# madeleineudell/LowRankModels.jl

Measured on AMD Instinct MI355X. Metric: observed-entry updates/sec, higher is better.
Workload: dtype f64

## Files before the change

### lowrankmodels.jl_amd/csrc/glrm_cached.hip

```cpp
#include <hip/hip_runtime.h>

#include <algorithm>
#include <atomic>
#include <vector>

#include "glrm_device.hpp"
#include "glrm_engine.hpp"
#include "glrm_launch.hpp"

using namespace glrm;

namespace {

struct CachedArgs {
  int64_t nseg;
  const int64_t* ptr;
  const int32_t* idx;
  const double* vals;
  double* own;
  int64_t own_offset;
  const double* other;
  double* alpha;
  const glrm_loss* losses;
  const glrm_reg* regs;
  int reg_single;
  int k;
  double fixed_alpha;
  double min_stepsize;
  int32_t* trials;
  int32_t* accepts;
  int cap;
  const int32_t* seglist;
  int64_t seg_lo, seg_hi;
  int vecreg;
};

__device__ __forceinline__ int64_t cached_segment(const CachedArgs& a, int64_t slot) {
  if (slot >= a.nseg) return -1;
  if (!a.seglist) return slot;
  const int64_t seg = a.seglist[slot];
  return (seg < a.seg_lo || seg >= a.seg_hi) ? -1 : seg;
}

template <int G, int R, int LOSS, bool GRAD>
__device__ __forceinline__ double cached_pass(const CachedArgs& a, const char* __restrict__ ybuf, const double* __restrict__ lval,
                                              const int32_t* __restrict__ lidx, const Vec<G, R>& xv, Vec<G, R>& g, int len, int gi, int j,
                                              const LossDesc& segloss) {
  constexpr int KPB = G * R * 8, NG = 64 / G, LM = loss_mode(LOSS), U = 4;
  constexpr bool TRIG = loss_trig(LOSS);
  double J = 0.0;
  if (GRAD) {
#pragma unroll
    for (int i = 0; i < R / 2; ++i) g.v[i] = make_double2(0.0, 0.0);
  }
  for (int t0 = 0; t0 < len; t0 += NG * U) {
    double2 y[U][R / 2];
    double av[U];
    int cc[U];
    bool valid[U];
#pragma unroll
    for (int u = 0; u < U; ++u) {
      const int t = t0 + u * NG + gi;
      valid[u] = t < len;
      const int tt = valid[u] ? t : len - 1;
      const char* yp = ybuf + tt * KPB + j * 16;
#pragma unroll
      for (int i = 0; i < R / 2; ++i) y[u][i] = *reinterpret_cast<const double2*>(yp + i * (G * 16));
      av[u] = lval[tt];
      cc[u] = lidx[tt];
    }
#pragma unroll
    for (int u = 0; u < U; ++u) {
      double dot = 0.0;
#pragma unroll
      for (int i = 0; i < R / 2; ++i) {
        dot = fma(xv.v[i].x, y[u][i].x, dot);
        dot = fma(xv.v[i].y, y[u][i].y, dot);
      }
      dot = group_sum<G>(dot);
      double L, dL;
      if constexpr (LOSS == LOSS_QUAD_UNIFORM) {
        const double d = dot - av[u];
        L = segloss.scale * (d * d);
        dL = 2 * d * segloss.scale;
      } else if constexpr (LM == LOSS_SEGMENT) {
        loss_both<GRAD, TRIG>(segloss, dot, av[u], L, dL);
      } else {
        const LossDesc lo = load_loss(a.losses, cc[u]);
        loss_both<GRAD, TRIG>(lo, dot, av[u], L, dL);
      }
      if (!valid[u]) {
        L = 0.0;
        dL = 0.0;
      }
      J += L;
      if (GRAD) {
#pragma unroll
        for (int i = 0; i < R / 2; ++i) {
          g.v[i].x = fma(dL, y[u][i].x, g.v[i].x);
          g.v[i].y = fma(dL, y[u][i].y, g.v[i].y);
        }
      }
    }
  }
  J = across_groups_sum<G>(J);
  if (GRAD) {
#pragma unroll
    for (int i = 0; i < R / 2; ++i) {
      g.v[i].x = across_groups_sum<G>(g.v[i].x);
      g.v[i].y = across_groups_sum<G>(g.v[i].y);
    }
  }
  return J;
}

template <int G, int R, int LOSS, bool VR = false>
__global__ void __launch_bounds__(64) cached_sweep_kernel(const CachedArgs a) {
  constexpr int KP = G * R, KPB = KP * 8, CPV = KPB / 16, VPI = 64 / CPV;
  extern __shared__ __attribute__((aligned(16))) char lds[];
  const int lane = threadIdx.x;
  const int64_t seg = cached_segment(a, blockIdx.x);
  if (seg < 0) return;
  const int j = lane % G, gi = lane / G;
  const int64_t beg = a.ptr[seg];
  const int len = (int)(a.ptr[seg + 1] - beg);
  const int64_t gseg = a.own_offset + seg;
  double2* ownp = reinterpret_cast<double2*>(a.own + gseg * KP);
  char* ybuf = lds;
  double* lval = reinterpret_cast<double*>(lds + (size_t)a.cap * KPB);
  int32_t* lidx = reinterpret_cast<int32_t*>(lds + (size_t)a.cap * (KPB + 8));

  for (int t = lane; t < len; t += 64) {
    lidx[t] = a.idx[beg + t];
    lval[t] = a.vals[beg + t];
  }
  __syncthreads();
  Vec<G, R> x, g;
#pragma unroll
  for (int i = 0; i < R / 2; ++i) x.v[i] = ownp[i * G + j];
  const RegDesc rd = load_reg(a.regs, a.reg_single ? 0 : seg);
  LossDesc segloss = LossDesc{0, 1.0, 0.0, 0.0};
  if constexpr (loss_mode(LOSS) != LOSS_PER_OBS) segloss = load_loss(a.losses, 0);
  const double alpha0 = a.alpha[seg];
  if (len > 0) {
    const int vsub = lane / CPV, chunk = lane % CPV;
    const char* obase = reinterpret_cast<const char*>(a.other) + chunk * 16;
    for (int it = 0; it * VPI < len; ++it) {
      int s = it * VPI + vsub;
      s = s < len ? s : len - 1;
      const char* src = obase + (int64_t)lidx[s] * KPB;
      __builtin_amdgcn_global_load_lds((const __attribute__((address_space(1))) void*)src,
                                       (__attribute__((address_space(3))) void*)(ybuf + it * 1024), 16, 0, 0);
    }
  }
  asm volatile("s_waitcnt vmcnt(0)" ::: "memory");
  __syncthreads();

  double Jold = cached_pass<G, R, LOSS, true>(a, ybuf, lval, lidx, x, g, len, gi, j, segloss);
  if (a.fixed_alpha > 0.0) {
    const double s = a.fixed_alpha / ((double)len + 1.0);
    Vec<G, R> xn;
#pragma unroll
    for (int i = 0; i < R / 2; ++i) {
      xn.v[i].x = x.v[i].x + g.v[i].x * (-s);
      xn.v[i].y = x.v[i].y + g.v[i].y * (-s);
    }
    reg_prox<G, R, VR>(rd, xn, s, j, a.k);
    if (gi == 0) {
#pragma unroll
      for (int i = 0; i < R / 2; ++i) ownp[i * G + j] = xn.v[i];
    }
    return;
  }
  Jold += reg_eval<G, R, VR>(rd, x, j, a.k);

  double alpha = alpha0;
  const double l = (double)len + 1.0;
  int ntrials = 0;
  bool accepted = false;
  while (alpha > a.min_stepsize) {
    const double s = alpha / l;
    Vec<G, R> xn, dummy;
#pragma unroll
    for (int i = 0; i < R / 2; ++i) {
      xn.v[i].x = fma(-s, g.v[i].x, x.v[i].x);
      xn.v[i].y = fma(-s, g.v[i].y, x.v[i].y);
    }
    reg_prox<G, R, VR>(rd, xn, s, j, a.k);
    double Jn = cached_pass<G, R, LOSS, false>(a, ybuf, lval, lidx, xn, dummy, len, gi, j, segloss);
    Jn += reg_eval<G, R, VR>(rd, xn, j, a.k);
    ++ntrials;
    if (Jn < Jold) {
      x = xn;
      alpha *= 1.05;
      Jold = Jn;
      accepted = true;
      break;
    }
    alpha *= .7;
    if (alpha < a.min_stepsize) {
      alpha = a.min_stepsize * 1.1;
      break;
    }
  }
  if (accepted && gi == 0) {
#pragma unroll
    for (int i = 0; i < R / 2; ++i) ownp[i * G + j] = x.v[i];
  }
  if (lane == 0) {
    a.alpha[seg] = alpha;
    if (a.trials) {
      a.trials[seg] += ntrials;
      a.accepts[seg] += accepted ? 1 : 0;
    }
  }
}

template <int G, int R, int LOSS, int MAXT, bool GRAD, int WAVES = 1>
__device__ __forceinline__ double reg_pass(const CachedArgs& a, const double2 (&y)[MAXT][R / 2], const double (&av)[MAXT], const int (&cc)[MAXT],
                                           const Vec<G, R>& xv, Vec<G, R>& g, int len, int gi, const LossDesc& segloss) {
  constexpr int NG = (64 / G) * WAVES, LM = loss_mode(LOSS);
  constexpr bool TRIG = loss_trig(LOSS);
  double J = 0.0;
  if (GRAD) {
#pragma unroll
    for (int i = 0; i < R / 2; ++i) g.v[i] = make_double2(0.0, 0.0);
  }
#pragma unroll
  for (int t = 0; t < MAXT; ++t) {
    if (t * NG + (gi & ~(64 / G - 1)) < len) {
      double dot = 0.0;
#pragma unroll
      for (int i = 0; i < R / 2; ++i) {
        dot = fma(xv.v[i].x, y[t][i].x, dot);
        dot = fma(xv.v[i].y, y[t][i].y, dot);
      }
      dot = group_sum<G>(dot);
      double L, dL;
      if constexpr (LOSS == LOSS_QUAD_UNIFORM) {
        const double d = dot - av[t];
        L = segloss.scale * (d * d);
        dL = 2 * d * segloss.scale;
      } else if constexpr (LM == LOSS_SEGMENT) {
        loss_both<GRAD, TRIG>(segloss, dot, av[t], L, dL);
      } else {
        const LossDesc lo = load_loss(a.losses, cc[t]);
        loss_both<GRAD, TRIG>(lo, dot, av[t], L, dL);
      }
      if (!(t * NG + gi < len)) {
        L = 0.0;
        dL = 0.0;
      }
      J += L;
      if (GRAD) {
#pragma unroll
        for (int i = 0; i < R / 2; ++i) {
          g.v[i].x = fma(dL, y[t][i].x, g.v[i].x);
          g.v[i].y = fma(dL, y[t][i].y, g.v[i].y);
        }
      }
    }
  }
  J = across_groups_sum<G>(J);
  if (GRAD) {
#pragma unroll
    for (int i = 0; i < R / 2; ++i) {
      g.v[i].x = across_groups_sum<G>(g.v[i].x);
      g.v[i].y = across_groups_sum<G>(g.v[i].y);
    }
  }
  return J;
}

template <int G, int R, int WAVES, bool GRAD>
__device__ __forceinline__ double row_combine(double J, Vec<G, R>& g, double* red, int wave, int lane) {
  constexpr int KP = G * R, STRIDE = KP + 2;
  if constexpr (WAVES == 1) return J;
  const int j = lane % G;
  __syncthreads();
  if (lane < G) {
    if (GRAD) {
#pragma unroll
      for (int i = 0; i < R / 2; ++i) *reinterpret_cast<double2*>(&red[wave * STRIDE + i * 2 * G + 2 * j]) = g.v[i];
    }
    if (lane == 0) red[wave * STRIDE + KP] = J;
  }
  __syncthreads();
  double Js = 0.0;
  if (GRAD) {
#pragma unroll
    for (int i = 0; i < R / 2; ++i) g.v[i] = make_double2(0.0, 0.0);
  }
  for (int w = 0; w < WAVES; ++w) {
    Js += red[w * STRIDE + KP];
    if (GRAD) {
#pragma unroll
      for (int i = 0; i < R / 2; ++i) {
        const double2 p = *reinterpret_cast<const double2*>(&red[w * STRIDE + i * 2 * G + 2 * j]);
        g.v[i].x += p.x;
        g.v[i].y += p.y;
      }
    }
  }
  return Js;
}

template <int G, int R, int LOSS, int MAXT, int WAVES, bool VR = false>
__global__ void __launch_bounds__(WAVES * 64) regcached_sweep_kernel(const CachedArgs a) {
  constexpr int KP = G * R, NG = (64 / G) * WAVES;
  __shared__ __attribute__((aligned(16))) double red[WAVES == 1 ? 2 : WAVES * (KP + 2)];
  const int lane = threadIdx.x & 63, wave = threadIdx.x >> 6;
  const int64_t seg = cached_segment(a, blockIdx.x);
  if (seg < 0) return;
  const int j = lane % G, gi = wave * (64 / G) + lane / G;
  const int64_t beg = a.ptr[seg];
  const int len = (int)(a.ptr[seg + 1] - beg);
  const int64_t gseg = a.own_offset + seg;
  double2* ownp = reinterpret_cast<double2*>(a.own + gseg * KP);
  int cc[MAXT];
  double av[MAXT];
  double2 y[MAXT][R / 2];
#pragma unroll
  for (int t = 0; t < MAXT; ++t) {
    int tt = t * NG + gi;
    tt = tt < len ? tt : (len > 0 ? len - 1 : 0);
    cc[t] = len > 0 ? a.idx[beg + tt] : 0;
    av[t] = len > 0 ? a.vals[beg + tt] : 0.0;
  }
  Vec<G, R> x, g;
#pragma unroll
  for (int i = 0; i < R / 2; ++i) x.v[i] = ownp[i * G + j];
  const double2* __restrict__ other2 = reinterpret_cast<const double2*>(a.other);
#pragma unroll
  for (int t = 0; t < MAXT; ++t) {
    if (t * NG + wave * (64 / G) < len) {
      const double2* yp = other2 + (int64_t)cc[t] * (KP / 2) + j;
#pragma unroll
      for (int i = 0; i < R / 2; ++i) y[t][i] = yp[i * G];
    } else {
#pragma unroll
      for (int i = 0; i < R / 2; ++i) y[t][i] = make_double2(0.0, 0.0);
    }
  }
  const RegDesc rd = load_reg(a.regs, a.reg_single ? 0 : seg);
  LossDesc segloss = LossDesc{0, 1.0, 0.0, 0.0};
  if constexpr (loss_mode(LOSS) != LOSS_PER_OBS) segloss = load_loss(a.losses, 0);

  double Jold = reg_pass<G, R, LOSS, MAXT, true, WAVES>(a, y, av, cc, x, g, len, gi, segloss);
  Jold = row_combine<G, R, WAVES, true>(Jold, g, red, wave, lane);
  if (a.fixed_alpha > 0.0) {
    const double s = a.fixed_alpha / ((double)len + 1.0);
    Vec<G, R> xn;
#pragma unroll
    for (int i = 0; i < R / 2; ++i) {
      xn.v[i].x = x.v[i].x + g.v[i].x * (-s);
      xn.v[i].y = x.v[i].y + g.v[i].y * (-s);
    }
    reg_prox<G, R, VR>(rd, xn, s, j, a.k);
    if (gi == 0) {
#pragma unroll
      for (int i = 0; i < R / 2; ++i) ownp[i * G + j] = xn.v[i];
    }
    return;
  }
  Jold += reg_eval<G, R, VR>(rd, x, j, a.k);
  double alpha = a.alpha[seg];
  const double l = (double)len + 1.0;
  int ntrials = 0;
  bool accepted = false;
  while (alpha > a.min_stepsize) {
    const double s = alpha / l;
    Vec<G, R> xn, dummy;
#pragma unroll
    for (int i = 0; i < R / 2; ++i) {
      xn.v[i].x = fma(-s, g.v[i].x, x.v[i].x);
      xn.v[i].y = fma(-s, g.v[i].y, x.v[i].y);
    }
    reg_prox<G, R, VR>(rd, xn, s, j, a.k);
    double Jn = reg_pass<G, R, LOSS, MAXT, false, WAVES>(a, y, av, cc, xn, dummy, len, gi, segloss);
    Jn = row_combine<G, R, WAVES, false>(Jn, dummy, red, wave, lane);
    Jn += reg_eval<G, R, VR>(rd, xn, j, a.k);
    ++ntrials;
    if (Jn < Jold) {
      x = xn;
      alpha *= 1.05;
      Jold = Jn;
      accepted = true;
      break;
    }
    alpha *= .7;
    if (alpha < a.min_stepsize) {
      alpha = a.min_stepsize * 1.1;
      break;
    }
  }
  if (accepted && gi == 0) {
#pragma unroll
    for (int i = 0; i < R / 2; ++i) ownp[i * G + j] = x.v[i];
  }
  if (lane == 0 && wave == 0) {
    a.alpha[seg] = alpha;
    if (a.trials) {
      a.trials[seg] += ntrials;
      a.accepts[seg] += accepted ? 1 : 0;
    }
  }
}

template <int G, int R, int LOSS, int MAXT, bool VR = false>
__global__ void __launch_bounds__(128, 2) regcached_persist_kernel(const CachedArgs a) {
  constexpr int WAVES = 2, KP = G * R, NG = (64 / G) * WAVES, MAXLEN = MAXT * NG, PF = (MAXLEN + 127) / 128;
  constexpr int RED = WAVES * (KP + 2);
  __shared__ __attribute__((aligned(16))) double sh[RED + PF * 128 + PF * 64];
  double* red = sh;
  double* lvals = sh + RED;
  int* lidx = reinterpret_cast<int*>(sh + RED + PF * 128);
  int* lvals_dw = reinterpret_cast<int*>(lvals);
  const int tid = threadIdx.x, lane = tid & 63, wave = tid >> 6;
  const int j = lane % G, gi = wave * (64 / G) + lane / G;
  const RegDesc rd0 = load_reg(a.regs, 0);
  LossDesc segloss = LossDesc{0, 1.0, 0.0, 0.0};
  if constexpr (loss_mode(LOSS) != LOSS_PER_OBS) segloss = load_loss(a.losses, 0);
  const double2* __restrict__ other2 = reinterpret_cast<const double2*>(a.other);

  auto seg_of = [&](int64_t slot) -> int64_t { return cached_segment(a, slot); };
  auto fetch_list = [&](int64_t beg, int len, int (&pi)[PF], int (&pv)[2 * PF]) {
#pragma unroll
    for (int q = 0; q < PF; ++q) {
      int e = q * 128 + tid;
      e = e < len ? e : (len > 0 ? len - 1 : 0);
      pi[q] = len > 0 ? a.idx[beg + e] : 0;
      const int2 v = len > 0 ? *reinterpret_cast<const int2*>(a.vals + beg + e) : make_int2(0, 0);
      pv[2 * q] = v.x; pv[2 * q + 1] = v.y;
    }
  };
  auto store_list = [&](const int (&pi)[PF], const int (&pv)[2 * PF]) {
#pragma unroll
    for (int q = 0; q < PF; ++q) {
      lidx[q * 128 + tid] = pi[q];
      lvals_dw[2 * (q * 128 + tid)] = pv[2 * q];
      lvals_dw[2 * (q * 128 + tid) + 1] = pv[2 * q + 1];
    }
  };

  int64_t slot = blockIdx.x;
  int64_t seg = seg_of(slot), seg_n = seg_of(slot + gridDim.x);
  int64_t beg = seg >= 0 ? a.ptr[seg] : 0, beg_n = seg_n >= 0 ? a.ptr[seg_n] : 0;
  int len = seg >= 0 ? (int)(a.ptr[seg + 1] - beg) : 0, len_n = seg_n >= 0 ? (int)(a.ptr[seg_n + 1] - beg_n) : 0;
  {
    int pi[PF], pv[2 * PF];
    fetch_list(beg, len, pi, pv);
    store_list(pi, pv);
  }
  __syncthreads();
  for (; slot < a.nseg; slot += gridDim.x) {
    const int64_t seg_nn = seg_of(slot + 2 * (int64_t)gridDim.x);
    const int64_t beg_nn = seg_nn >= 0 ? a.ptr[seg_nn] : 0;
    const int len_nn = seg_nn >= 0 ? (int)(a.ptr[seg_nn + 1] - beg_nn) : 0;
    int cc[MAXT];
    double av[MAXT];
    double2 y[MAXT][R / 2];
#pragma unroll
    for (int t = 0; t < MAXT; ++t) {
      int tt = t * NG + gi;
      tt = tt < len ? tt : (len > 0 ? len - 1 : 0);
      cc[t] = lidx[tt];
      av[t] = lvals[tt];
    }
    const int64_t gseg = a.own_offset + (seg >= 0 ? seg : 0);
    double2* ownp = reinterpret_cast<double2*>(a.own + gseg * KP);
    Vec<G, R> x, g;
#pragma unroll
    for (int i = 0; i < R / 2; ++i) x.v[i] = ownp[i * G + j];
#pragma unroll
    for (int t = 0; t < MAXT; ++t) {
      if (t * NG + wave * (64 / G) < len) {
        const double2* yp = other2 + (int64_t)cc[t] * (KP / 2) + j;
#pragma unroll
        for (int i = 0; i < R / 2; ++i) y[t][i] = yp[i * G];
      } else {
#pragma unroll
        for (int i = 0; i < R / 2; ++i) y[t][i] = make_double2(0.0, 0.0);
      }
    }
    int pi[PF], pv[2 * PF];
    fetch_list(beg_n, len_n, pi, pv);
    const RegDesc rd = a.reg_single ? rd0 : load_reg(a.regs, seg >= 0 ? seg : 0);

    if (seg >= 0) {
      double Jold = reg_pass<G, R, LOSS, MAXT, true, WAVES>(a, y, av, cc, x, g, len, gi, segloss);
      Jold = row_combine<G, R, WAVES, true>(Jold, g, red, wave, lane);
      if (a.fixed_alpha > 0.0) {
        const double s = a.fixed_alpha / ((double)len + 1.0);
        Vec<G, R> xn;
#pragma unroll
        for (int i = 0; i < R / 2; ++i) {
          xn.v[i].x = x.v[i].x + g.v[i].x * (-s);
          xn.v[i].y = x.v[i].y + g.v[i].y * (-s);
        }
        reg_prox<G, R, VR>(rd, xn, s, j, a.k);
        if (gi == 0) {
#pragma unroll
          for (int i = 0; i < R / 2; ++i) ownp[i * G + j] = xn.v[i];
        }
      } else {
        Jold += reg_eval<G, R, VR>(rd, x, j, a.k);
        double alpha = a.alpha[seg];
        const double l = (double)len + 1.0;
        int ntrials = 0;
        bool accepted = false;
        while (alpha > a.min_stepsize) {
          const double s = alpha / l;
          Vec<G, R> xn, dummy;
#pragma unroll
          for (int i = 0; i < R / 2; ++i) {
            xn.v[i].x = fma(-s, g.v[i].x, x.v[i].x);
            xn.v[i].y = fma(-s, g.v[i].y, x.v[i].y);
          }
          reg_prox<G, R, VR>(rd, xn, s, j, a.k);
          double Jn = reg_pass<G, R, LOSS, MAXT, false, WAVES>(a, y, av, cc, xn, dummy, len, gi, segloss);
          Jn = row_combine<G, R, WAVES, false>(Jn, dummy, red, wave, lane);
          Jn += reg_eval<G, R, VR>(rd, xn, j, a.k);
          ++ntrials;
          if (Jn < Jold) {
            x = xn;
            alpha *= 1.05;
            Jold = Jn;
            accepted = true;
            break;
          }
          alpha *= .7;
          if (alpha < a.min_stepsize) {
            alpha = a.min_stepsize * 1.1;
            break;
          }
        }
        if (accepted && gi == 0) {
#pragma unroll
          for (int i = 0; i < R / 2; ++i) ownp[i * G + j] = x.v[i];
        }
        if (tid == 0) {
          a.alpha[seg] = alpha;
          if (a.trials) {
            a.trials[seg] += ntrials;
            a.accepts[seg] += accepted ? 1 : 0;
          }
        }
      }
    }
    __syncthreads();
    store_list(pi, pv);
    __syncthreads();
    seg = seg_n; beg = beg_n; len = len_n;
    seg_n = seg_nn; beg_n = beg_nn; len_n = len_nn;
  }
}

template <int G, int R, int LOSS, bool VR>
int launch_reg_inst(const CachedArgs& a, hipStream_t st, glrm_handle* h) {
  const int waves = env_int("GLRM_HIP_CACHED_WAVES", 2);
  if (waves == 2 && env_int("GLRM_HIP_CACHED_PERSIST", 1)) {
    const bool small = (a.cap + 1) / 2 <= 4;
    int& cache = h->cached_grid[(small ? 1 : 0) + (VR ? 2 : 0)];
    int nb = cache;
    if (nb == 0) {
      int per_cu = 0;
      hipDeviceProp_t prop;
      const void* k = small ? (const void*)regcached_persist_kernel<G, R, LOSS, 4, VR> : (const void*)regcached_persist_kernel<G, R, LOSS, 7, VR>;
      if (hipOccupancyMaxActiveBlocksPerMultiprocessor(&per_cu, k, 128, 0) != hipSuccess || per_cu < 1) { (void)hipGetLastError(); per_cu = 1; }
      int cus = 256;
      if (hipGetDeviceProperties(&prop, h->device) == hipSuccess && prop.multiProcessorCount > 0) cus = prop.multiProcessorCount;
      nb = per_cu * cus;
      if (nb < 1) nb = 1;
      cache = nb;
    }
    const unsigned grid = (unsigned)std::min<int64_t>(a.nseg, nb);
    if (small) hipLaunchKernelGGL((regcached_persist_kernel<G, R, LOSS, 4, VR>), dim3(grid), dim3(128), 0, st, a);
    else hipLaunchKernelGGL((regcached_persist_kernel<G, R, LOSS, 7, VR>), dim3(grid), dim3(128), 0, st, a);
    return GLRM_OK;
  }
  if (waves == 4 && (a.cap + 3) / 4 <= 4) {
    hipLaunchKernelGGL((regcached_sweep_kernel<G, R, LOSS, 4, 4, VR>), dim3((unsigned)a.nseg), dim3(256), 0, st, a);
  } else if (waves == 1) {
    if (a.cap <= 7) hipLaunchKernelGGL((regcached_sweep_kernel<G, R, LOSS, 7, 1, VR>), dim3((unsigned)a.nseg), dim3(64), 0, st, a);
    else hipLaunchKernelGGL((regcached_sweep_kernel<G, R, LOSS, 13, 1, VR>), dim3((unsigned)a.nseg), dim3(64), 0, st, a);
  } else if ((a.cap + 1) / 2 <= 4) {
    hipLaunchKernelGGL((regcached_sweep_kernel<G, R, LOSS, 4, 2, VR>), dim3((unsigned)a.nseg), dim3(128), 0, st, a);
  } else {
    hipLaunchKernelGGL((regcached_sweep_kernel<G, R, LOSS, 7, 2, VR>), dim3((unsigned)a.nseg), dim3(128), 0, st, a);
  }
  return GLRM_OK;
}

template <int G, int R, int LOSS, bool VR>
int launch_inst(const CachedArgs& a, hipStream_t st) {
  const int lds = a.cap * (G * R * 8 + 12);
  if (lds > 65536)
    HIPCK(hipFuncSetAttribute(reinterpret_cast<const void*>(cached_sweep_kernel<G, R, LOSS, VR>), hipFuncAttributeMaxDynamicSharedMemorySize, lds));
  hipLaunchKernelGGL((cached_sweep_kernel<G, R, LOSS, VR>), dim3((unsigned)a.nseg), dim3(64), lds, st, a);
  return GLRM_OK;
}

}

int glrm_setup_cached(glrm_handle* h) {
  h->cached_row = h->cached_want = 0;
  const int want = env_int("GLRM_HIP_CACHED", h->tiled_opt == 1 ? 0 : -1);
  if (want == 0 || h->tiled_row || h->sig.nnz_rows <= 0) return GLRM_OK;
  if (!((h->G == 4 || h->G == 8) && h->R == 8)) return GLRM_OK;
  if (want < 0) {
    const double opp_bytes = (double)h->n * h->kp * 8;
    if (opp_bytes <= 32.0 * 1024 * 1024 || (double)h->sig.nnz_rows < 1e8) return GLRM_OK;
  }
  h->cached_want = 1;
  h->cached_row = env_int("GLRM_HIP_CACHED_REGS", 1) ? 2 : 1;
  return GLRM_OK;
}

int64_t glrm_cached_maxlen(const glrm_handle* h) {
  if (h->cached_row == 2) return glrm_cached_reg_maxlen(h->G);
  const int vpi = 64 / (h->kp * 8 / 16);
  const int64_t budget = env_int("GLRM_HIP_CACHED", -1) > 0 ? 160 * 1024 : 53 * 1024;
  return budget / (h->kp * 8 + 12) / vpi * vpi;
}

void glrm_cached_set_cap(glrm_handle* h, int64_t maxlen) {
  if (h->cached_row == 2) {
    const int ng = 64 / h->G;
    h->cached_cap = (int)((maxlen + ng - 1) / ng);
  } else {
    const int vpi = 64 / (h->kp * 8 / 16);
    h->cached_cap = (int)((maxlen + vpi - 1) / vpi * vpi);
    if (h->cached_cap < vpi) h->cached_cap = vpi;
  }
}

int glrm_run_cached(glrm_handle* h, int loss, double min_stepsize, const int32_t* seglist, int64_t nlist, hipStream_t st) {
  CachedArgs a{};
  glrm_fill_side(a, h, true, min_stepsize, 0);
  a.cap = h->cached_cap;
  a.seg_lo = 0;
  a.seg_hi = h->ml;
  if (seglist) {
    a.seglist = seglist;
    a.nseg = nlist;
    if (h->rng_e >= 0) { a.seg_lo = h->rng_b; a.seg_hi = h->rng_e; }
    if (a.nseg <= 0 || a.seg_hi <= a.seg_lo) return GLRM_OK;
  } else if (h->rng_e >= 0) {
    glrm_apply_row_range(a, h->rng_b, h->rng_e);
    if (a.nseg <= 0) return GLRM_OK;
  }
  auto by_layout = [&](auto g, auto r) {
    constexpr int G = decltype(g)::value, R = decltype(r)::value;
    auto by_loss = [&](auto LOSS) {
      constexpr int L = decltype(LOSS)::value;
      if (a.vecreg) return h->cached_row == 2 ? launch_reg_inst<G, R, L, true>(a, st, h) : launch_inst<G, R, L, true>(a, st);
      return h->cached_row == 2 ? launch_reg_inst<G, R, L, false>(a, st, h) : launch_inst<G, R, L, false>(a, st);
    };
    return glrm_dispatch<LOSS_QUAD_UNIFORM, LOSS_SEGMENT, LOSS_SEGMENT_NOTRIG, LOSS_PER_OBS_NOTRIG>(loss, by_loss, [&] { return by_loss(glrm_const<LOSS_PER_OBS>{}); });
  };
  const int rc = glrm_dispatch_layout<32>(h->G, 8, by_layout, [&] { return by_layout(glrm_const<8>{}, glrm_const<8>{}); });
  if (rc) return rc;
  HIPCK(hipGetLastError());
  return GLRM_OK;
}
```

Before: 10.55 billion.

## Double-buffer segment lists in LDS and prefetch alpha with the next record

The persistent kernel now keeps two shared-memory buffers for the segment index/value list and writes the next segment's list into the alternate buffer during the current segment's work. This removes one block-wide barrier per iteration. The step size alpha is prefetched along with the list, and the pointer reads go through the constant address space. The change doubles LDS use, which may lower occupancy, and it replaces the trial counter updates with atomics.

```diff
diff --git a/lowrankmodels.jl_amd/csrc/glrm_cached.hip b/lowrankmodels.jl_amd/csrc/glrm_cached.hip
--- a/lowrankmodels.jl_amd/csrc/glrm_cached.hip
+++ b/lowrankmodels.jl_amd/csrc/glrm_cached.hip
@@ -410,12 +410,9 @@
 template <int G, int R, int LOSS, int MAXT, bool VR = false>
 __global__ void __launch_bounds__(128, 2) regcached_persist_kernel(const CachedArgs a) {
   constexpr int WAVES = 2, KP = G * R, NG = (64 / G) * WAVES, MAXLEN = MAXT * NG, PF = (MAXLEN + 127) / 128;
-  constexpr int RED = WAVES * (KP + 2);
-  __shared__ __attribute__((aligned(16))) double sh[RED + PF * 128 + PF * 64];
+  constexpr int RED = WAVES * (KP + 2), REC = PF * 128 + 128 + PF * 64;
+  __shared__ __attribute__((aligned(16))) double sh[RED + 2 * REC];
   double* red = sh;
-  double* lvals = sh + RED;
-  int* lidx = reinterpret_cast<int*>(sh + RED + PF * 128);
-  int* lvals_dw = reinterpret_cast<int*>(lvals);
   const int tid = threadIdx.x, lane = tid & 63, wave = tid >> 6;
   const int j = lane % G, gi = wave * (64 / G) + lane / G;
   const RegDesc rd0 = load_reg(a.regs, 0);
@@ -423,8 +420,18 @@
   if constexpr (loss_mode(LOSS) != LOSS_PER_OBS) segloss = load_loss(a.losses, 0);
   const double2* __restrict__ other2 = reinterpret_cast<const double2*>(a.other);
 
-  auto seg_of = [&](int64_t slot) -> int64_t { return cached_segment(a, slot); };
-  auto fetch_list = [&](int64_t beg, int len, int (&pi)[PF], int (&pv)[2 * PF]) {
+  const auto* kptr = (const __attribute__((address_space(4))) int64_t*)a.ptr;
+  const auto* klist = (const __attribute__((address_space(4))) int32_t*)a.seglist;
+  auto seg_of = [&](int64_t slot) -> int64_t {
+    if (slot >= a.nseg) return -1;
+    if (!a.seglist) return slot;
+    const int64_t s = klist[slot];
+    return (s < a.seg_lo || s >= a.seg_hi) ? -1 : s;
+  };
+  auto rec_vals = [&](int buf) -> double* { return sh + RED + buf * REC; };
+  auto rec_alpha = [&](int buf) -> double* { return sh + RED + buf * REC + PF * 128; };
+  auto rec_idx = [&](int buf) -> int* { return reinterpret_cast<int*>(sh + RED + buf * REC + PF * 128 + 128); };
+  auto fetch_rec = [&](int64_t sg, int64_t beg, int len, int (&pi)[PF], int (&pv)[2 * PF], double& pa) {
 #pragma unroll
     for (int q = 0; q < PF; ++q) {
       int e = q * 128 + tid;
@@ -433,63 +440,85 @@
       const int2 v = len > 0 ? *reinterpret_cast<const int2*>(a.vals + beg + e) : make_int2(0, 0);
       pv[2 * q] = v.x; pv[2 * q + 1] = v.y;
     }
+    pa = a.alpha[sg >= 0 ? sg : 0];
   };
-  auto store_list = [&](const int (&pi)[PF], const int (&pv)[2 * PF]) {
+  auto store_rec = [&](int buf, const int (&pi)[PF], const int (&pv)[2 * PF], double pa) {
+    int* li = rec_idx(buf);
+    int* lv = reinterpret_cast<int*>(rec_vals(buf));
 #pragma unroll
     for (int q = 0; q < PF; ++q) {
-      lidx[q * 128 + tid] = pi[q];
-      lvals_dw[2 * (q * 128 + tid)] = pv[2 * q];
-      lvals_dw[2 * (q * 128 + tid) + 1] = pv[2 * q + 1];
-    }
+      li[q * 128 + tid] = pi[q];
+      lv[2 * (q * 128 + tid)] = pv[2 * q];
+      lv[2 * (q * 128 + tid) + 1] = pv[2 * q + 1];
+    }
+    rec_alpha(buf)[tid] = pa;
   };
 
   int64_t slot = blockIdx.x;
   int64_t seg = seg_of(slot), seg_n = seg_of(slot + gridDim.x);
-  int64_t beg = seg >= 0 ? a.ptr[seg] : 0, beg_n = seg_n >= 0 ? a.ptr[seg_n] : 0;
-  int len = seg >= 0 ? (int)(a.ptr[seg + 1] - beg) : 0, len_n = seg_n >= 0 ? (int)(a.ptr[seg_n + 1] - beg_n) : 0;
+  int64_t beg = seg >= 0 ? kptr[seg] : 0, beg_n = seg_n >= 0 ? kptr[seg_n] : 0;
+  int len = seg >= 0 ? (int)(kptr[seg + 1] - beg) : 0, len_n = seg_n >= 0 ? (int)(kptr[seg_n + 1] - beg_n) : 0;
   {
     int pi[PF], pv[2 * PF];
-    fetch_list(beg, len, pi, pv);
-    store_list(pi, pv);
+    double pa;
+    fetch_rec(seg, beg, len, pi, pv, pa);
+    store_rec(0, pi, pv, pa);
   }
   __syncthreads();
+  int cur = 0;
   for (; slot < a.nseg; slot += gridDim.x) {
-    const int64_t seg_nn = seg_of(slot + 2 * (int64_t)gridDim.x);
-    const int64_t beg_nn = seg_nn >= 0 ? a.ptr[seg_nn] : 0;
-    const int len_nn = seg_nn >= 0 ? (int)(a.ptr[seg_nn + 1] - beg_nn) : 0;
-    int cc[MAXT];
-    double av[MAXT];
-    double2 y[MAXT][R / 2];
-#pragma unroll
-    for (int t = 0; t < MAXT; ++t) {
-      int tt = t * NG + gi;
-      tt = tt < len ? tt : (len > 0 ? len - 1 : 0);
-      cc[t] = lidx[tt];
-      av[t] = lvals[tt];
-    }
-    const int64_t gseg = a.own_offset + (seg >= 0 ? seg : 0);
-    double2* ownp = reinterpret_cast<double2*>(a.own + gseg * KP);
-    Vec<G, R> x, g;
-#pragma unroll
-    for (int i = 0; i < R / 2; ++i) x.v[i] = ownp[i * G + j];
-#pragma unroll
-    for (int t = 0; t < MAXT; ++t) {
-      if (t * NG + wave * (64 / G) < len) {
-        const double2* yp = other2 + (int64_t)cc[t] * (KP / 2) + j;
-#pragma unroll
-        for (int i = 0; i < R / 2; ++i) y[t][i] = yp[i * G];
-      } else {
-#pragma unroll
-        for (int i = 0; i < R / 2; ++i) y[t][i] = make_double2(0.0, 0.0);
-      }
-    }
-    int pi[PF], pv[2 * PF];
-    fetch_list(beg_n, len_n, pi, pv);
-    const RegDesc rd = a.reg_single ? rd0 : load_reg(a.regs, seg >= 0 ? seg : 0);
-
-    if (seg >= 0) {
+    int64_t seg_nn, beg_nn;
+    int len_nn;
+    auto next_pointers = [&] {
+      seg_nn = seg_of(slot + 2 * (int64_t)gridDim.x);
+      const int64_t p0 = kptr[seg_nn >= 0 ? seg_nn : 0], p1 = kptr[(seg_nn >= 0 ? seg_nn : 0) + 1];
+      beg_nn = seg_nn >= 0 ? p0 : 0;
+      len_nn = seg_nn >= 0 ? (int)(p1 - p0) : 0;
+    };
+    if (seg < 0) {
+      int pi[PF], pv[2 * PF];
+      double pa;
+      fetch_rec(seg_n, beg_n, len_n, pi, pv, pa);
+      next_pointers();
+      store_rec(cur ^ 1, pi, pv, pa);
+    } else {
+      const double* lvals = rec_vals(cur);
+      const int* lidx = rec_idx(cur);
+      int cc[MAXT];
+      double av[MAXT];
+      double2 y[MAXT][R / 2];
+#pragma unroll
+      for (int t = 0; t < MAXT; ++t) {
+        int tt = t * NG + gi;
+        tt = tt < len ? tt : (len > 0 ? len - 1 : 0);
+        cc[t] = lidx[tt];
+        av[t] = lvals[tt];
+      }
+      const int64_t gseg = a.own_offset + seg;
+      double2* ownp = reinterpret_cast<double2*>(a.own + gseg * KP);
+      Vec<G, R> x, g;
+#pragma unroll
+      for (int i = 0; i < R / 2; ++i) x.v[i] = ownp[i * G + j];
+#pragma unroll
+      for (int t = 0; t < MAXT; ++t) {
+        if (t * NG + wave * (64 / G) < len) {
+          const double2* yp = other2 + (int64_t)cc[t] * (KP / 2) + j;
+#pragma unroll
+          for (int i = 0; i < R / 2; ++i) y[t][i] = yp[i * G];
+        } else {
+#pragma unroll
+          for (int i = 0; i < R / 2; ++i) y[t][i] = make_double2(0.0, 0.0);
+        }
+      }
+      int pi[PF], pv[2 * PF];
+      double pa;
+      fetch_rec(seg_n, beg_n, len_n, pi, pv, pa);
+      next_pointers();
+      const RegDesc rd = a.reg_single ? rd0 : load_reg(a.regs, seg);
+
       double Jold = reg_pass<G, R, LOSS, MAXT, true, WAVES>(a, y, av, cc, x, g, len, gi, segloss);
       Jold = row_combine<G, R, WAVES, true>(Jold, g, red, wave, lane);
+      store_rec(cur ^ 1, pi, pv, pa);
       if (a.fixed_alpha > 0.0) {
         const double s = a.fixed_alpha / ((double)len + 1.0);
         Vec<G, R> xn;
@@ -505,7 +534,7 @@
         }
       } else {
         Jold += reg_eval<G, R, VR>(rd, x, j, a.k);
-        double alpha = a.alpha[seg];
+        double alpha = rec_alpha(cur)[tid];
         const double l = (double)len + 1.0;
         int ntrials = 0;
         bool accepted = false;
@@ -542,15 +571,14 @@
         if (tid == 0) {
           a.alpha[seg] = alpha;
           if (a.trials) {
-            a.trials[seg] += ntrials;
-            a.accepts[seg] += accepted ? 1 : 0;
+            atomicAdd(&a.trials[seg], ntrials);
+            atomicAdd(&a.accepts[seg], accepted ? 1 : 0);
           }
         }
       }
     }
     __syncthreads();
-    store_list(pi, pv);
-    __syncthreads();
+    cur ^= 1;
     seg = seg_n; beg = beg_n; len = len_n;
     seg_n = seg_nn; beg_n = beg_nn; len_n = len_nn;
   }
```

After: 10.96 billion, median of 6. +3.8%, better.
